# choutilin/makani

Hardware: AMD Instinct MI355X
Metric: SFNO fwd+bwd samples/sec, 73ch 721x1440 (higher is better)
Workload: dtype bf16; 1 GPU; sfno_linear_73chq_sc3_layers8_edim384 fwd+bwd+Adam, 73ch 721x1440, per-GPU batch 1; global_batch=1, parallelism=h1, spectral_dtype=f32 (GEMMs as 6 bf16 MFMA products of exact 3-way operand splits), step_launch=eager, micro_batches=1, python_gc=disabled in the timed region, adam=after backward

## Files before the change

### include/makani_amd.h

```cpp
#ifndef MAKANI_AMD_H
#define MAKANI_AMD_H

#include <stdint.h>

#ifdef __cplusplus
extern "C" {
#endif

int mk_version(void);
const char* mk_last_error(void);


int mk_quadrature(int grid, int nlat, double* theta, double* weights);

int mk_legendre_kpad(int nlat);

int mk_legendre_table(int grid, int nlat, int lmax, int mmax, int with_quad_weights, float* out);

int mk_fft_twiddle_len(int nlon);
int mk_fft_twiddles(int nlon, float* out);

int mk_rfft(const void* x, int x_dtype, float* xf, const float* twiddles,
            int bc, int nlat, int nlon, int mmax, float scale0, float scale_m, float scale_h,
            void* stream);
// ... 23 lines not shown
                          int mmax_loc, int m_off, int mmax_glob, int xf_layout, void* stream);
int mk_legendre_inv_x3_ex(const float* c, const void* tab_x3, float* xf, int bc, int nlat, int lmax,
                          int mmax_loc, int m_off, int mmax_glob, int xf_layout, void* stream);

int mk_rfft_pm(const void* x, int x_dtype, float* xf, const float* twiddles, int bc, int nlat, int nlon, int mmax,
               float scale0, float scale_m, float scale_h, int chans, int chans_per_peer, void* stream);
int mk_irfft_pm(const float* xf, void* x, int x_dtype, const float* twiddles, int bc, int nlat, int nlon, int mmax,
                float scale0, float scale_m, float scale_h, int chans, int chans_per_peer, void* stream);

int mk_irfft_sums(const float* xf, void* x, int x_dtype, const float* twiddles, int bc, int nlat, int nlon, int mmax,
                  float scale0, float scale_m, float scale_h, int xf_layout, int chans, int chans_per_peer, double* rowsums,
                  void* stream);
int mk_irfft_affine_add(const float* xf, void* x, int x_dtype, const float* twiddles, int bc, int nlat, int nlon,
                        int mmax, float scale0, float scale_m, float scale_h, int xf_layout, const void* z,
                        const float* affine, void* stream);

int mk_dhconv_fwd(const float* x, const float* w, float* y, int lloc, int mloc, int batch,
                  int cin, int cout, int l_off, int m_off, void* stream);
int mk_dhconv_dgrad(const float* gy, const float* w, float* gx, int lloc, int mloc, int batch,
                    int cin, int cout, int l_off, int m_off, void* stream);
int mk_dhconv_wgrad(const float* x, const float* gy, float* gw, int lloc, int mloc, int batch,
                    int cin, int cout, int l_off, int m_off, void* stream);

int mk_dhconv_fwd_x3(const float* x, const float* w, float* y, int lloc, int mloc, int batch,
                     int cin, int cout, int l_off, int m_off, void* stream);
int mk_dhconv_dgrad_x3(const float* gy, const float* w, float* gx, int lloc, int mloc, int batch,
                       int cin, int cout, int l_off, int m_off, void* stream);
int mk_dhconv_wgrad_x3(const float* x, const float* gy, float* gw, int lloc, int mloc, int batch,
                       int cin, int cout, int l_off, int m_off, void* stream);

// ... 117 lines not shown
```

### makani_amd/_lib.py

```python
import ctypes
import os

import torch

from . import build as _build

_LIB = None

_c_int = ctypes.c_int
_c_float = ctypes.c_float
_vp = ctypes.c_void_p

SIGNATURES = {
    "mk_version": (_c_int, []),
    "mk_last_error": (ctypes.c_char_p, []),
    "mk_quadrature": (_c_int, [_c_int, _c_int, _vp, _vp]),
    "mk_legendre_kpad": (_c_int, [_c_int]),
    "mk_legendre_table": (_c_int, [_c_int, _c_int, _c_int, _c_int, _c_int, _vp]),
    "mk_fft_twiddle_len": (_c_int, [_c_int]),
    "mk_fft_twiddles": (_c_int, [_c_int, _vp]),
    "mk_rfft": (_c_int, [_vp, _c_int, _vp, _vp, _c_int, _c_int, _c_int, _c_int, _c_float, _c_float, _c_float, _vp]),
    "mk_irfft": (_c_int, [_vp, _vp, _c_int, _vp, _c_int, _c_int, _c_int, _c_int, _c_float, _c_float, _c_float, _vp]),
    "mk_legendre_fwd": (_c_int, [_vp, _vp, _vp, _c_int, _c_int, _c_int, _c_int, _c_int, _c_int, _vp]),
    "mk_legendre_inv": (_c_int, [_vp, _vp, _vp, _c_int, _c_int, _c_int, _c_int, _c_int, _c_int, _vp]),
    "mk_legendre_x3_bytes": (ctypes.c_longlong, [_c_int, _c_int, _c_int, _c_int]),
    "mk_legendre_x3_split": (_c_int, [_vp, _vp, _c_int, _c_int, _c_int, _c_int, _vp]),
    "mk_legendre_fwd_x3": (_c_int, [_vp, _vp, _vp, _c_int, _c_int, _c_int, _c_int, _c_int, _c_int, _vp]),
    "mk_legendre_inv_x3": (_c_int, [_vp, _vp, _vp, _c_int, _c_int, _c_int, _c_int, _c_int, _c_int, _vp]),
    "mk_rfft_ex": (_c_int, [_vp, _c_int, _vp, _vp, _c_int, _c_int, _c_int, _c_int, _c_float, _c_float, _c_float, _c_int, _vp]),
    "mk_irfft_ex": (_c_int, [_vp, _vp, _c_int, _vp, _c_int, _c_int, _c_int, _c_int, _c_float, _c_float, _c_float, _c_int, _vp]),
    "mk_rfft_pm": (_c_int, [_vp, _c_int, _vp, _vp, _c_int, _c_int, _c_int, _c_int, _c_float, _c_float, _c_float, _c_int, _c_int, _vp]),
    "mk_irfft_pm": (_c_int, [_vp, _vp, _c_int, _vp, _c_int, _c_int, _c_int, _c_int, _c_float, _c_float, _c_float, _c_int, _c_int, _vp]),
    "mk_irfft_sums": (_c_int, [_vp, _vp, _c_int, _vp, _c_int, _c_int, _c_int, _c_int, _c_float, _c_float, _c_float, _c_int, _c_int,
                               _c_int, _vp, _vp]),
    "mk_irfft_affine_add": (_c_int, [_vp, _vp, _c_int, _vp, _c_int, _c_int, _c_int, _c_int, _c_float, _c_float, _c_float, _c_int,
                                     _vp, _vp, _vp]),
    "mk_legendre_fwd_x3_ex": (_c_int, [_vp, _vp, _vp, _c_int, _c_int, _c_int, _c_int, _c_int, _c_int, _c_int, _vp]),
    "mk_legendre_inv_x3_ex": (_c_int, [_vp, _vp, _vp, _c_int, _c_int, _c_int, _c_int, _c_int, _c_int, _c_int, _vp]),
    "mk_dhconv_fwd": (_c_int, [_vp, _vp, _vp] + [_c_int] * 7 + [_vp]),
    "mk_dhconv_dgrad": (_c_int, [_vp, _vp, _vp] + [_c_int] * 7 + [_vp]),
    "mk_dhconv_wgrad": (_c_int, [_vp, _vp, _vp] + [_c_int] * 7 + [_vp]),
    "mk_dhconv_fwd_x3": (_c_int, [_vp, _vp, _vp] + [_c_int] * 7 + [_vp]),
    "mk_dhconv_dgrad_x3": (_c_int, [_vp, _vp, _vp] + [_c_int] * 7 + [_vp]),
    "mk_dhconv_wgrad_x3": (_c_int, [_vp, _vp, _vp] + [_c_int] * 7 + [_vp]),
    "mk_spec_mix_fwd": (_c_int, [_vp, _vp, _vp] + [_c_int] * 7 + [_vp]),
    "mk_spec_mix_dgrad": (_c_int, [_vp, _vp, _vp] + [_c_int] * 7 + [_vp]),
    "mk_spec_mix_wgrad": (_c_int, [_vp, _vp, _vp] + [_c_int] * 7 + [_vp]),
    "mk_affine_add": (_c_int, [_vp, _vp, _vp, _vp, _c_int, _c_int, ctypes.c_longlong, _vp]),
    "mk_diag_fwd": (_c_int, [_vp, _vp, _vp, _c_int, _c_int, _c_int, ctypes.c_longlong, _vp]),
    "mk_diag_dgrad": (_c_int, [_vp, _vp, _vp, _c_int, _c_int, _c_int, ctypes.c_longlong, _vp]),
    "mk_diag_wgrad": (_c_int, [_vp, _vp, _vp, _c_int, _c_int, _c_int, ctypes.c_longlong, _vp]),
# ... 92 lines not shown
```

### makani_amd/build.py

```python
import os
import shutil
import subprocess
import sys

HERE = os.path.dirname(os.path.abspath(__file__))
CSRC = os.path.join(HERE, "csrc")
LIB = os.path.join(HERE, "libmakani_amd.so")
STAMP = LIB + ".stamp"
SOURCES = ["host.cpp", "fft.hip", "gemm.hip", "gemm_x3.hip", "layout.hip", "diag.hip", "pointwise.hip", "conv_gemm.hip", "pce.hip", "pce_mlp.hip", "adam.hip", "optim.hip", "metrics.hip", "lploss.hip", "preproc.hip", "zenith.hip"]
HEADERS = ["common.h", "fft_split.h", "lds_dma.h", "pce_common.h", os.path.join("..", "..", "include", "makani_amd.h")]


def _hipcc():
    for cand in (shutil.which("hipcc"), "/opt/rocm/bin/hipcc"):
        if cand and os.path.exists(cand):
            return cand
    raise RuntimeError("hipcc not found; libmakani_amd.so cannot be built")


def have_hipcc():
    return any(c and os.path.exists(c) for c in (shutil.which("hipcc"), "/opt/rocm/bin/hipcc"))


def _source_digest():
    import hashlib
# ... 54 lines not shown
```

### makani_amd/csrc/fft.hip

```cpp
#include "common.h"
#include "../../include/makani_amd.h"

#include <hip/hip_bf16.h>
#include <cstdint>
#include <cstdlib>
#include <type_traits>
#include <utility>

namespace {

struct XfLayout {
    int sm, sk;
    int C, Cp, Bn;
    long long pstride;
};
static thread_local XfLayout g_xl = {0, 0, 0, 0, 0, 0};
static thread_local const void* g_addz = nullptr;
static thread_local const float* g_affine = nullptr;
static thread_local double* g_rowsums = nullptr;

struct XfChan {
    size_t pbase;
    int bcx0, BCx;
};
__device__ __forceinline__ XfChan xf_chan(const XfLayout& xl, int bc0, int BC) {
    XfChan c{0, bc0, BC};
    if (xl.Cp) {
        const int b = bc0 / xl.C, ch = bc0 - b * xl.C, pp = ch / xl.Cp;
        c.pbase = (size_t)pp * (size_t)xl.pstride;
        c.bcx0 = b * xl.Cp + (ch - pp * xl.Cp);
        c.BCx = xl.Bn * xl.Cp;
    }
    return c;
}


template <int I>
using IC = std::integral_constant<int, I>;

template <class F, int... Is>
__device__ __forceinline__ void static_for_impl(F&& f, std::integer_sequence<int, Is...>) {
    (f(IC<Is>{}), ...);
}
template <int N, class F>
__device__ __forceinline__ void static_for(F&& f) {
    static_for_impl(static_cast<F&&>(f), std::make_integer_sequence<int, N>{});
}

constexpr double kPi = 3.14159265358979323846264338327950288;

constexpr double cx_reduce(double x) {
    while (x > kPi) x -= 2.0 * kPi;
    while (x < -kPi) x += 2.0 * kPi;
    return x;
}
constexpr double cx_sin(double x) {
    x = cx_reduce(x);
    double term = x, sum = x;
    for (int n = 1; n < 20; ++n) {
        term *= -x * x / ((2.0 * n) * (2.0 * n + 1.0));
        sum += term;
    }
// ... 526 lines not shown
extern "C" int mk_irfft_affine_add(const float* xf, void* x, int x_dtype, const float* twiddles, int bc, int nlat, int nlon,
                                   int mmax, float scale0, float scale_m, float scale_h, int xf_layout, const void* z,
                                   const float* affine, void* stream) {
    MK_REQUIRE(z != nullptr && affine != nullptr, "null pointer");
    MK_REQUIRE(!fft_legacy() && mmax <= 241 && (nlon == 480 || nlon == 1440), "the affine-add epilogue exists in the split kernels only");
    MK_REQUIRE((((uintptr_t)z | (uintptr_t)x) & 15) == 0, "fields must be 16-byte aligned");
    MK_REQUIRE(xf_layout == 0 || xf_layout == 1, "xf_layout must be 0 ([M][K][BC]) or 1 ([K][M][BC])");
    MK_REQUIRE((240LL * (xf_layout ? 1 : nlat) + 1) * bc * 8 < (1LL << 31), "Fourier rows too large for the 32-bit gather offsets");
    g_addz = z;
    g_affine = affine;
    const int rc = mk_irfft_ex(xf, x, x_dtype, twiddles, bc, nlat, nlon, mmax, scale0, scale_m, scale_h, xf_layout, stream);
    g_addz = nullptr;
    g_affine = nullptr;
    return rc;
}
```

### makani_amd/csrc/fft_split.h

```cpp

constexpr int SH = 240;
constexpr int SP = 272;
constexpr int SNSUB = 24;
constexpr int STHREADS = 384;
constexpr int SLDS_F2 = SNSUB * SP + 96;

__device__ __forceinline__ int pair_tile(int i) {
    const int xcd = i & 7, seq = i >> 3;
    return ((((seq >> 1) << 3) + xcd) << 1) + (seq & 1);
}

__device__ __forceinline__ int sub_base(int sr, int S) { return sr * SP + 4 * (sr / S); }
__device__ __forceinline__ int phi(int i) { return i + (i >> 4); }
__device__ __forceinline__ int opaque(int v) {
    asm volatile("" : "+v"(v));
    return v;
}

template <typename T> __device__ __forceinline__ float as_stored(float v);
template <> __device__ __forceinline__ float as_stored<float>(float v) { return v; }
template <> __device__ __forceinline__ float as_stored<__hip_bfloat16>(float v) { return __bfloat162float(__float2bfloat16(v)); }

template <bool SUMS = false, typename TOut = float>
__device__ __forceinline__ void split_passes(float2* lds, int tid, int S, const float2 (&tw15)[15], float* red = nullptr) {
// ... 206 lines not shown
        const unsigned int w[4] = {u.x, u.y, u.z, u.w};
#pragma unroll
        for (int i = 0; i < 4; ++i) {
            o[2 * i] = __uint_as_float(w[i] << 16);
            o[2 * i + 1] = __uint_as_float(w[i] & 0xffff0000u);
        }
    }
    static __device__ __forceinline__ void store(__hip_bfloat16* p, const float (&o)[8]) {
        __hip_bfloat16 h[8];
#pragma unroll
        for (int i = 0; i < 8; ++i) h[i] = __float2bfloat16(o[i]);
        *reinterpret_cast<uint4*>(p) = *reinterpret_cast<const uint4*>(h);
    }
};

template <int S, typename TOut, bool WIDE, int PERSIST, bool SUMS = false, bool ADD = false>
__global__ __launch_bounds__(STHREADS, PERSIST ? 3 : 5) void irfft_split_kernel(const float2* __restrict__ xf, TOut* __restrict__ x,
                                                               const float2* __restrict__ tw, int BC, int K, int M,
                                                               float scale0, float scale_m, float scale_h, XfLayout xl,
                                                               double* __restrict__ rowsums, const TOut* __restrict__ addz,
                                                               const float* __restrict__ affine) {
    constexpr int N = 480 * S, G = SNSUB / S, HH = N / 2;
    extern __shared__ __attribute__((aligned(16))) float2 lds[];
    float* red = reinterpret_cast<float*>(lds + SLDS_F2);
    const int tid = threadIdx.x;
    const int ntile = (BC + G - 1) / G;
    const int total = ntile * K;
    const float2* tw2 = tw + HH;
    const int total16 = (total + 15) & ~15;
    auto next_valid = [&](int i) {
        while (i < total16 && pair_tile(i) >= total) i += (int)gridDim.x;
        return i;
    };
    int sched = PERSIST ? next_valid(blockIdx.x) : (int)blockIdx.x;
    if (sched >= total16) return;
    int tile = pair_tile(sched);
    if (!PERSIST && tile >= total) return;
// ... 42 lines not shown
#pragma unroll
            for (int it = 0; it < PIT; ++it) {
                const int jp = jp0 + STEP * it, j1 = SH - jp;
                const bool oa = chan_ok && jp < NPAIR && jp < M, ob = chan_ok && jp < NPAIR && j1 < M;
                xa[it] = *(oa ? base + (size_t)jp * xl.sm * xc.BCx : xf);
                xb[it] = *(ob ? base + (size_t)j1 * xl.sm * xc.BCx : xf);
            }
        }
    };
    gather(tile, tid);
  for (;;) {
    const int tl = opaque(tid);
    const int k = tile / ntile, bc0 = (tile - k * ntile) * G;
    const int jp0 = tl / G, g = tl - jp0 * G;
    const bool chan_ok = bc0 + g < BC;
#pragma unroll
    for (int it = 0; it < PIT; ++it) {
        const int jp = jp0 + STEP * it;
        if (jp >= NPAIR) continue;
        const int j1 = SH - jp;
        const float sa = (chan_ok && jp < M) ? ((jp == 0) ? scale0 : scale_m) : 0.f;
        const float sb = (chan_ok && j1 < M) ? ((j1 == HH) ? scale_h : scale_m) : 0.f;
        const float2 a0 = make_float2(sa * xa[it].x, sa * xa[it].y);
        const float2 b0 = make_float2(sb * xb[it].x, sb * xb[it].y);
        float2 wsub = it ? cmul(wfirst[0], tw2[S * STEP * it]) : wfirst[0];
        wsub.y = -wsub.y;
#pragma unroll
        for (int s = 0; s < S; ++s) {
            float2 ya = a0, yb = b0;
            if (s > 0) {
// ... 45 lines not shown
                const float2* zs = lds + sub_base(g * S + sq, S) + phi((EO / 2) * p);
#pragma unroll
                for (int h = 0; h < EO / 2; ++h) {
                    const float2 z = zs[h];
                    r[sq][2 * h] = z.x;
                    r[sq][2 * h + 1] = -z.y;
                }
            }
            const size_t doff = ((size_t)(bc0 + g) * K + k) * N + (size_t)p * EO * S;
            TOut* dst = x + doff;
            float za[S][EO];
            float ca = 0.f, cb = 0.f;
            if constexpr (ADD) {
                ca = affine[2 * (bc0 + g)];
                cb = affine[2 * (bc0 + g) + 1];
#pragma unroll
                for (int c = 0; c < S; ++c) OutVec<TOut>::load(addz + doff + c * EO, za[c]);
            }
#pragma unroll
            for (int c = 0; c < S; ++c) {
                float o[EO];
#pragma unroll
                for (int e = 0; e < EO; ++e) {
                    const int f = c * EO + e;
                    o[e] = r[f % S][f / S];
                    if constexpr (ADD) o[e] += fmaf(za[c][e], ca, cb);
                }
                OutVec<TOut>::store(dst + c * EO, o);
            }
        }
    }
    if (next >= total16) break;
    sched = next;
    tile = pair_tile(next);
    __syncthreads();
  }
}

static inline unsigned split_grid(long long tiles) { return (unsigned)((tiles + 15) / 16 * 16); }

static inline int fft_exp() {
    static const int v = [] { const char* e = getenv("MK_FFT_EXP"); return e ? atoi(e) : 0; }();
    return v;
}

// ... 12 lines not shown
    return 0;
}

template <int S>
int launch_irfft_split(const float* xf, void* x, int x_dtype, const float* tw, int bc, int nlat, int mmax, float s0,
                       float sm, float sh, hipStream_t st) {
    constexpr int G = SNSUB / S;
    const dim3 grid(split_grid(mk::ceil_div(bc, G) * (long long)nlat));
    const size_t lds = sizeof(float2) * SLDS_F2 + 2 * SNSUB * sizeof(float);
    const long long bcx = g_xl.Cp ? (long long)g_xl.Bn * g_xl.Cp : (long long)bc;
    const bool wide = ((long long)SH * g_xl.sm + 1) * bcx * 8 >= (1LL << 31);
#define MK_IRFFT_LAUNCH(T, W, PS, SM)                                                                                  \
    hipLaunchKernelGGL((irfft_split_kernel<S, T, W, PS, SM>), grid, dim3(STHREADS), lds, st, (const float2*)xf, (T*)x,    \
                       (const float2*)tw, bc, nlat, mmax, s0, sm, sh, g_xl, g_rowsums, (const T*)nullptr, (const float*)nullptr)
#define MK_IRFFT_PICK(T)                                                                                               \
    if (g_addz) {                                                                                                      \
        if (wide) return -1;                                                                                           \
        hipLaunchKernelGGL((irfft_split_kernel<S, T, false, 0, false, true>), grid, dim3(STHREADS), lds, st,           \
                           (const float2*)xf, (T*)x, (const float2*)tw, bc, nlat, mmax, s0, sm, sh, g_xl, nullptr,     \
                           (const T*)g_addz, g_affine);                                                                \
    } else if (g_rowsums) {                                                                                                   \
        if (wide) MK_IRFFT_LAUNCH(T, true, 1, true); else MK_IRFFT_LAUNCH(T, false, 0, true);                          \
    } else {                                                                                                           \
        if (wide) MK_IRFFT_LAUNCH(T, true, 1, false); else MK_IRFFT_LAUNCH(T, false, 0, false);                        \
    }
    if (x_dtype == 0) {
        MK_IRFFT_PICK(float)
    } else {
        MK_IRFFT_PICK(__hip_bfloat16)
    }
#undef MK_IRFFT_PICK
// ... 12 lines not shown
```

### makani_amd/csrc/pointwise.hip

```cpp
#include "common.h"
#include "../../include/makani_amd.h"

#include <hip/hip_bf16.h>

namespace {

constexpr int kT = 256;
constexpr int kE = 8;
constexpr int kSteps = 4;
constexpr int kChunk = kT * kE * kSteps;

template <typename T> struct IO;
template <> struct IO<float> {
    static __device__ __forceinline__ void load(const float* p, float (&v)[kE]) {
        const float4 a = reinterpret_cast<const float4*>(p)[0], b = reinterpret_cast<const float4*>(p)[1];
        v[0] = a.x; v[1] = a.y; v[2] = a.z; v[3] = a.w; v[4] = b.x; v[5] = b.y; v[6] = b.z; v[7] = b.w;
    }
    static __device__ __forceinline__ void store(float* p, const float (&v)[kE]) {
        reinterpret_cast<float4*>(p)[0] = make_float4(v[0], v[1], v[2], v[3]);
        reinterpret_cast<float4*>(p)[1] = make_float4(v[4], v[5], v[6], v[7]);
    }
    static __device__ __forceinline__ float ld1(const float* p) { return *p; }
    static __device__ __forceinline__ void st1(float* p, float v) { *p = v; }
};
// ... 5 lines not shown
        for (int i = 0; i < 4; ++i) {
            v[2 * i] = __uint_as_float(w[i] << 16);
            v[2 * i + 1] = __uint_as_float(w[i] & 0xffff0000u);
        }
    }
    static __device__ __forceinline__ void store(__hip_bfloat16* p, const float (&v)[kE]) {
        __hip_bfloat16 h[kE];
#pragma unroll
        for (int i = 0; i < kE; ++i) h[i] = __float2bfloat16(v[i]);
        *reinterpret_cast<uint4*>(p) = *reinterpret_cast<const uint4*>(h);
    }
    static __device__ __forceinline__ float ld1(const __hip_bfloat16* p) { return __bfloat162float(*p); }
    static __device__ __forceinline__ void st1(__hip_bfloat16* p, float v) { *p = __float2bfloat16(v); }
};

struct PhiPair {
    float Phi, phi;
};
__device__ __forceinline__ PhiPair normal_cdf_pdf_fast(float x) {
    const float z = fabsf(x) * 0.70710678118654752f;
    const float t = __builtin_amdgcn_rcpf(fmaf(0.3275911f, z, 1.0f));
    float q = fmaf(1.061405429f, t, -1.453152027f);
    q = fmaf(q, t, 1.421413741f);
    q = fmaf(q, t, -0.284496736f);
    q = fmaf(q, t, 0.254829592f);
    const float e = __builtin_amdgcn_exp2f(-1.4426950408889634f * z * z);
    const float half_erfc = 0.5f * q * t * e;
    PhiPair r;
    r.Phi = x < 0.f ? half_erfc : 1.0f - half_erfc;
    r.phi = 0.3989422804014327f * e;
    return r;
}
template <typename T> struct Act;
template <> struct Act<float> {
    static __device__ __forceinline__ float gelu(float z) { return 0.5f * z * (1.f + erff(z * 0.70710678118654752440f)); }
    static __device__ __forceinline__ float gelu_grad(float z) {
        return 0.5f * (1.f + erff(z * 0.70710678118654752440f)) + z * 0.39894228040143267794f * __expf(-0.5f * z * z);
    }
};
template <> struct Act<__hip_bfloat16> {
    static __device__ __forceinline__ float gelu(float z) { return z * normal_cdf_pdf_fast(z).Phi; }
    static __device__ __forceinline__ float gelu_grad(float z) {
        const PhiPair c = normal_cdf_pdf_fast(z);
        return fmaf(z, c.phi, c.Phi);
    }
};

template <typename T, class F>
__device__ __forceinline__ void for_chunk(long long P, F&& f) {
    const long long c0 = (long long)blockIdx.x * kChunk;
#pragma unroll
    for (int s = 0; s < kSteps; ++s) {
        const long long off = c0 + ((long long)s * kT + threadIdx.x) * kE;
        if (off + kE <= P)
            f(off, kE);
        else if (off < P)
            f(off, (int)(P - off));
    }
}

__device__ __forceinline__ float block_sum(float v, float* red) {
// ... 481 lines not shown
```

### makani_amd/layers.py

```python
import math
import os

import torch
import torch.nn as nn
import torch.nn.functional as F
from torch.utils.checkpoint import checkpoint


class _X3Conv(torch.autograd.Function):

    @staticmethod
    def forward(ctx, x3, w, addend):
        from . import ops
        wf = w.detach().float()
        ctx.save_for_backward(x3, wf)
        ctx.cfg = (w.dtype, addend is not None)
        return ops.conv1x1_x3(wf, x3, out=None if addend is None else addend.detach())

    @staticmethod
    def backward(ctx, gy):
        from . import ops
        x3, wf = ctx.saved_tensors
        wdt, has_addend = ctx.cfg
        gy = gy.contiguous()
# ... 287 lines not shown
        from . import ops
        x3, w, pre = ctx.saved_tensors
        (wimg_t, gbuf), ctx.step = (ctx.step or (None, None)), None
        need_gb = ctx.bias_dtype is not None and ctx.needs_input_grad[2]
        gpre, gsum = ops.gelu_backward(pre, gh.contiguous(), need_gb)
        gx = gw = gb = None
        if ctx.needs_input_grad[0]:
            gx = ops.pce_gemm(gpre, wimg_t if wimg_t is not None else ops.pce_pack(w, transpose=True), w.shape[1])
        if ctx.needs_input_grad[1]:
            gw = ops.conv1x1_wgrad_raw(gpre, x3, out=gbuf).to(w.dtype)
        if need_gb:
            gb = gsum.to(ctx.bias_dtype)
        return gx, gw, gb, None


def encoder_head(encoder, x):
    from . import ops
    mods = list(encoder.fwd)
    pat = _mlp_pattern(mods)
    if pat is None or x.dim() != 4:
        return None
    fc1, fc2 = pat
    if fc2.bias is not None or not ops.spec_mix_supported(fc2.in_channels, fc2.out_channels):
        return None
    x3 = _engine_field(x)
    if x3 is None or not ops.pce_supported_train(fc1.out_channels, fc1.in_channels):
        return None
    with torch.autocast("cuda", enabled=False):
        h = _PceConvGelu.apply(x3, fc1.weight2d(), fc1.bias, torch.is_grad_enabled())
    return h.view(x.shape[0], fc1.out_channels, x.shape[2], x.shape[3]), fc2


class _PceMLP(torch.autograd.Function):

    @staticmethod
    def forward(ctx, x3, w1, b1, w2, b2, apply_b2, want_row_sums, keep_pre=True):
        from . import ops
        if keep_pre:
            h, pre = ops.pce_gemm(x3, ops.pce_pack(w1), w1.shape[0], bias=b1, want_pre=True, gelu=True)
        else:
            h, pre = ops.pce_gemm(x3, ops.pce_pack(w1), w1.shape[0], bias=b1, gelu=True), x3.new_empty(0)
        want_row_sums = bool(want_row_sums) and w2.shape[0] <= 768
# ... 385 lines not shown
```

### makani_amd/ops.py

```python
import ctypes
import math
import os

import numpy as np
import torch

from . import _lib

GRIDS = {"equiangular": 0, "legendre-gauss": 1}


def _stream():
    return torch.cuda.current_stream().cuda_stream


def _need_cuda(*tensors):
    for t in tensors:
        if not t.is_cuda:
            raise RuntimeError("makani_amd: the spectral ops run only on a HIP device (got a CPU tensor); "
                               "there is no CPU fallback")


def quadrature(grid, nlat):
    if grid not in GRIDS:
# ... 63 lines not shown
    else:
        m, k, bc = xf.shape
    x = torch.empty(bc, k, nlon, dtype=out_dtype, device=xf.device)
    sums = torch.zeros(bc, 2, dtype=torch.float64, device=xf.device)
    _lib.check(_lib.load().mk_irfft_sums(xf.data_ptr(), x.data_ptr(), 1 if out_dtype == torch.bfloat16 else 0, twiddles.data_ptr(),
                                         bc, k, nlon, m, 1.0, 1.0, 1.0, int(bool(kmajor)), int(chans), int(cpp), sums.data_ptr(),
                                         _stream()), "mk_irfft_sums")
    return x, sums


def irfft_affine_add_supported(nlon, mmax):
    return nlon in (480, 1440) and mmax <= 241 and os.environ.get("MK_FFT_LEGACY", "0") != "1" \
        and os.environ.get("MK_IRFFT_AFFINE_ADD", "1") != "0"


def irfft_affine_add_raw(xf, twiddles, nlon, z, affine, kmajor=False):
    _need_cuda(xf, twiddles, z, affine)
    assert xf.dim() == 3 and xf.is_contiguous() and xf.dtype == torch.complex64
    if kmajor:
        k, m, bc = xf.shape
    else:
        m, k, bc = xf.shape
    assert z.is_contiguous() and z.numel() == bc * k * nlon and z.dtype in (torch.float32, torch.bfloat16)
    assert affine.dtype == torch.float32 and affine.is_contiguous() and affine.numel() == 2 * bc
    x = torch.empty_like(z)
    _lib.check(_lib.load().mk_irfft_affine_add(xf.data_ptr(), x.data_ptr(), _pw_dtype(z), twiddles.data_ptr(), bc, k, nlon, m,
                                               1.0, 1.0, 1.0, int(bool(kmajor)), z.data_ptr(), affine.data_ptr(), _stream()),
               "mk_irfft_affine_add")
    return x


def irfft_raw(xf, twiddles, nlon, s0, sm, sh, out_dtype=torch.float32, kmajor=False):
    _need_cuda(xf, twiddles)
    assert xf.dim() == 3 and xf.is_contiguous() and xf.dtype == torch.complex64
    if kmajor:
        k, m, bc = xf.shape
    else:
        m, k, bc = xf.shape
    fused = out_dtype == torch.bfloat16 and irfft_bf16_rows(nlon, m)
    x = torch.empty(bc, k, nlon, dtype=torch.bfloat16 if fused else torch.float32, device=xf.device)
    _lib.check(_lib.load().mk_irfft_ex(xf.data_ptr(), x.data_ptr(), 1 if fused else 0, twiddles.data_ptr(), bc, k, nlon, m,
                                       s0, sm, sh, int(bool(kmajor)), _stream()), "mk_irfft")
    return x if x.dtype == out_dtype else x.to(out_dtype)

# ... 472 lines not shown
        ctx.save_for_backward(twiddles)
        ctx.nlon = x.shape[-1]
        ctx.in_dtype = x.dtype
        ctx.kmajor = kmajor
        s = 2.0 * math.pi / ctx.nlon
        return rfft_raw(x, twiddles, mmax, s, s, s, kmajor)

    @staticmethod
    def backward(ctx, gxf):
        (tw,) = ctx.saved_tensors
        n = ctx.nlon
        gx = irfft_raw(gxf.contiguous(), tw, n, 2.0 * math.pi / n, math.pi / n, 2.0 * math.pi / n, ctx.in_dtype, ctx.kmajor)
        return gx, None, None, None


class _IRFFT(torch.autograd.Function):

    @staticmethod
    def forward(ctx, xf, twiddles, nlon, out_dtype, kmajor=False, want_sums=False):
        ctx.save_for_backward(twiddles)
        ctx.mmax = xf.shape[1] if kmajor else xf.shape[0]
        ctx.kmajor = kmajor
        if want_sums:
            x, sums = irfft_sums_raw(xf, twiddles, nlon, out_dtype, kmajor)
            ctx.mark_non_differentiable(sums)
            return x, sums
        return irfft_raw(xf, twiddles, nlon, 1.0, 1.0, 1.0, out_dtype, kmajor)

    @staticmethod
    def backward(ctx, gx, *_):
# ... 165 lines not shown
        gy = gy.contiguous()
        gx = gw = None
        if ctx.needs_input_grad[0]:
            gx = spec_mix_dgrad_raw(gy, wf.view(wf.shape[0], -1), batch, l_off, m_off)
        if ctx.needs_input_grad[1]:
            gw = spec_mix_wgrad_raw(x, gy, batch, l_off, m_off).view(wshape).to(wdt)
        return gx, gw, None, None, None


def spec_mix(x, w, batch, l_off=0, m_off=0):
    return _SpecMix.apply(x, w, batch, l_off, m_off)


def rfft(x, twiddles, mmax, kmajor=False):
    return _RFFT.apply(x, twiddles, mmax, kmajor)


def irfft(xf, twiddles, nlon, out_dtype=torch.float32, kmajor=False, want_sums=False):
    return _IRFFT.apply(xf, twiddles, nlon, out_dtype, kmajor, want_sums)


def rfft_pm(x, twiddles, mmax, chans, cpp):
    return _RFFTpm.apply(x, twiddles, mmax, chans, cpp)


def irfft_pm(xf, twiddles, nlon, out_dtype, chans, cpp, want_sums=False):
    return _IRFFTpm.apply(xf, twiddles, nlon, out_dtype, chans, cpp, want_sums)


def legendre_fwd(xf, table, lmax, m_off=0, kmajor=False):
# ... 426 lines not shown
```

### makani_amd/sfnonet.py

```python
import math
import os
from functools import partial

import torch
import torch.nn as nn
import torch.nn.functional as F
from torch.utils.checkpoint import checkpoint

from . import comm
from .distributed import DistributedInverseRealFFT2, DistributedInverseRealSHT, DistributedRealFFT2, DistributedRealSHT
from .layer_norm import DistributedInstanceNorm2d, DistributedLayerNorm
from .layers import (Conv1x1, DropPath, EncoderDecoder, InstanceNorm2d, InverseRealFFT2, MLP, RealFFT2, _engine_field,
                     _is_exact_gelu, _is_noop, conv_plus_instance_norm, encoder_head, spectral_skip_plus_instance_norm,
                     spectral_skip_supported)
from .sht import InverseRealSHT, RealSHT
from .spectral_convolution import FactorizedSpectralConv, SpectralAttention, SpectralConv

_ACTIVATIONS = {"relu": nn.ReLU, "gelu": nn.GELU, "silu": nn.SiLU}


def _local_shape(transform):
    if comm.get_size("spatial") > 1:
        return transform.lat_shapes[comm.get_rank("h")], transform.lon_shapes[comm.get_rank("w")]
    return transform.nlat, transform.nlon
# ... 274 lines not shown
    def _forward_features(self, x, premix=None):
        for _ in range(self.repeat_layers):
            for i, blk in enumerate(self.blocks):
                if i == 0 and premix is not None:
                    x = blk(x, premix=premix)
                else:
                    x = checkpoint(blk, x, use_reentrant=False) if self.checkpointing >= 3 else blk(x)
        return x

    def _spectral_encoder(self, x):
        blk = self.blocks[0] if len(self.blocks) else None
        if (blk is None or hasattr(self, "pos_embed") or not _is_noop(self.pos_drop) or self.checkpointing != 0
                or self.repeat_layers != 1 or not blk.filter.takes_spectral_mix() or not blk.filter.filter.scale_residual
                or hasattr(blk, "inner_skip")):
            return None
        return encoder_head(self.encoder, x)

    def _engine_arena(self, x):
        from . import ops
        from .layers import Conv1x1
        if not (x.is_cuda and x.dim() == 4 and os.environ.get("MK_ENGINE_ARENA", "1") != "0"):
            return None
        if not (x.dtype == torch.bfloat16 or (torch.is_autocast_enabled() and torch.get_autocast_dtype("cuda") == torch.bfloat16)):
            return None
        cached = self.__dict__.get("_arena")
        if cached is None:
            convs = [m for m in self.modules() if isinstance(m, Conv1x1)]
        else:
            convs = cached[0]
        ptrs = [m.weight.data_ptr() for m in convs]
        if cached is None or cached[1] != ptrs:
# ... 35 lines not shown
```

### makani_amd/sht.py

```python
import torch
import torch.nn as nn

from . import ops


class _SHTBase(nn.Module):
    def __init__(self, nlat, nlon, lmax=None, mmax=None, grid="legendre-gauss", norm="ortho", csphase=True):
        super().__init__()
        if norm != "ortho" or not csphase:
            raise NotImplementedError("only norm='ortho', csphase=True (what Makani uses) are built")
        if grid not in ops.GRIDS:
            raise ValueError(f"Unknown quadrature mode {grid}")
        if nlon % 2:
            raise ValueError("nlon must be even")
        self.nlat, self.nlon, self.grid = nlat, nlon, grid
        self.norm, self.csphase = norm, csphase
        self.lmax = lmax or nlat
        self.mmax = mmax or nlon // 2 + 1
        if self.mmax > nlon // 2 + 1:
            raise ValueError("mmax exceeds nlon // 2 + 1")
        self.register_buffer("twiddles", ops.fft_twiddles(nlon), persistent=False)

    def _flatten(self, x, inner):
        lead = x.shape[:-2]
        bc = 1
        for s in lead:
            bc *= s
        return lead, x.reshape(bc, *inner)

    def extra_repr(self):
        return f"nlat={self.nlat}, nlon={self.nlon}, lmax={self.lmax}, mmax={self.mmax}, grid={self.grid}"


class RealSHT(_SHTBase):

    def __init__(self, nlat, nlon, lmax=None, mmax=None, grid="legendre-gauss", norm="ortho", csphase=True):
        super().__init__(nlat, nlon, lmax, mmax, grid, norm, csphase)
        self.register_buffer("weights", ops.legendre_table(grid, nlat, self.lmax, self.mmax, True), persistent=False)

    def forward_packed(self, x3):
        km = ops.SPECTRAL_GEMM == "bf16x3"
        xf = ops.rfft(x3, self.twiddles, self.mmax, km)
        return ops.legendre_fwd(xf, self.weights, self.lmax, 0, km)

    def forward(self, x):
        if x.shape[-2] != self.nlat or x.shape[-1] != self.nlon:
            raise ValueError(f"expected [..., {self.nlat}, {self.nlon}], got {tuple(x.shape)}")
        if x.dtype not in (torch.float32, torch.bfloat16):
            x = x.float()
        lead, x3 = self._flatten(x.contiguous(), (self.nlat, self.nlon))
        c = ops.spec_unpack(self.forward_packed(x3), 0, 0)
        return c.reshape(*lead, self.lmax, self.mmax)


class InverseRealSHT(_SHTBase):

    def __init__(self, nlat, nlon, lmax=None, mmax=None, grid="legendre-gauss", norm="ortho", csphase=True):
# ... 21 lines not shown
```

### makani_amd/spectral_convolution.py

```python
import math

import torch
import torch.nn as nn

from . import comm, ops
from .contractions import get_contract_fun
from .distributed import DistributedInverseRealFFT2, DistributedInverseRealSHT, DistributedRealSHT
from .sht import InverseRealSHT, RealSHT


def _is_hip_pair(fwd, inv):
    return isinstance(fwd, (RealSHT, DistributedRealSHT)) and isinstance(inv, (InverseRealSHT, DistributedInverseRealSHT))


class SpectralConv(nn.Module):
    def __init__(self, forward_transform, inverse_transform, in_channels, out_channels, operator_type="diagonal",
                 separable=False, bias=False, gain=1.0):
        super().__init__()
        self.forward_transform = forward_transform
        self.inverse_transform = inverse_transform
        self.in_channels = in_channels
        self.out_channels = out_channels
        self.modes_lat = self.inverse_transform.lmax
        self.modes_lon = self.inverse_transform.mmax
# ... 69 lines not shown
    def synthesise(self, c, B, odt):
        it = self.inverse_transform
        return it.inverse_packed(c, B, odt) if self._distributed else it.inverse_packed(c, odt)

    def residual_from_spectrum(self, c, B, dtype):
        with torch.autocast(device_type="cuda", enabled=False):
            r = self.synthesise(c, B, dtype if dtype in (torch.float32, torch.bfloat16) else torch.float32)
        return r.view(B, -1, r.shape[-2], r.shape[-1]).to(dtype)

    def takes_spectral_mix(self):
        return type(self) is SpectralConv and self._fused

    def _forward_fused(self, x, dtype, want_row_sums=False, premix=None, spectrum_residual=False):
        B, C = x.shape[0], x.shape[1]
        ft, it = self.forward_transform, self.inverse_transform
        xin = x if x.dtype in (torch.float32, torch.bfloat16) else x.float()
        xin = xin.contiguous()
        if isinstance(ft, DistributedRealSHT):
            c = ft.forward_packed(xin)
        else:
            c = ft.forward_packed(xin.view(B * C, xin.shape[2], xin.shape[3]))
        if premix is not None:
            c = ops.spec_mix(c, premix.weight, B, self.l_off, self.m_off)
            C = premix.out_channels
        odt = dtype if dtype in (torch.float32, torch.bfloat16) else torch.float32
        residual = x
        if self.scale_residual and spectrum_residual:
            residual = c
        elif self.scale_residual:
            r = self.synthesise(c, B, odt)
            residual = r.view(B, C, r.shape[-2], r.shape[-1]).to(dtype)
        y = ops.dhconv(c, self._weight_tensor(), B, self.l_off, self.m_off)
        sums = None
        if want_row_sums:
            out, sums = it.inverse_packed(y, B, odt, True) if self._distributed else it.inverse_packed(y, odt, True)
        else:
# ... 188 lines not shown
```

Measured before the change: 24.18 samples/s.

## Fuse encoder GELU gradient into iRFFT epilogue and fork RFFT skip-gradient add

Adds an iRFFT split-kernel epilogue that multiplies the synthesized gradient by the GELU derivative of the saved pre-activation and reduces per-channel bias-gradient sums. The encoder head's first conv+GELU output then feeds the first block's RFFT directly, and the backward produces gpre in one pass instead of a separate iRFFT, GELU-backward and bias reduction. A second path, rfft_fork, folds the residual skip gradient into the iRFFT via the existing affine-add epilogue for non-rescaling blocks. This saves full-resolution field reads and writes and some launches, at the cost of more template instantiations and extra per-workgroup atomics.

```diff
diff --git a/include/makani_amd.h b/include/makani_amd.h
--- a/include/makani_amd.h
+++ b/include/makani_amd.h
@@ -61,6 +61,8 @@
 int mk_irfft_affine_add(const float* xf, void* x, int x_dtype, const float* twiddles, int bc, int nlat, int nlon,
                         int mmax, float scale0, float scale_m, float scale_h, int xf_layout, const void* z,
                         const float* affine, void* stream);
+int mk_irfft_gelu_mul(const float* xf, const void* pre, void* gpre, double* rowsums, int x_dtype, const float* twiddles, int bc,
+                      int nlat, int nlon, int mmax, float scale0, float scale_m, float scale_h, int xf_layout, void* stream);
 
 int mk_dhconv_fwd(const float* x, const float* w, float* y, int lloc, int mloc, int batch,
                   int cin, int cout, int l_off, int m_off, void* stream);
diff --git a/makani_amd/_lib.py b/makani_amd/_lib.py
--- a/makani_amd/_lib.py
+++ b/makani_amd/_lib.py
@@ -35,6 +35,8 @@
                                _c_int, _vp, _vp]),
     "mk_irfft_affine_add": (_c_int, [_vp, _vp, _c_int, _vp, _c_int, _c_int, _c_int, _c_int, _c_float, _c_float, _c_float, _c_int,
                                      _vp, _vp, _vp]),
+    "mk_irfft_gelu_mul": (_c_int, [_vp, _vp, _vp, _vp, _c_int, _vp, _c_int, _c_int, _c_int, _c_int, _c_float, _c_float, _c_float,
+                                   _c_int, _vp]),
     "mk_legendre_fwd_x3_ex": (_c_int, [_vp, _vp, _vp, _c_int, _c_int, _c_int, _c_int, _c_int, _c_int, _c_int, _vp]),
     "mk_legendre_inv_x3_ex": (_c_int, [_vp, _vp, _vp, _c_int, _c_int, _c_int, _c_int, _c_int, _c_int, _c_int, _vp]),
     "mk_dhconv_fwd": (_c_int, [_vp, _vp, _vp] + [_c_int] * 7 + [_vp]),
diff --git a/makani_amd/build.py b/makani_amd/build.py
--- a/makani_amd/build.py
+++ b/makani_amd/build.py
@@ -8,7 +8,7 @@
 LIB = os.path.join(HERE, "libmakani_amd.so")
 STAMP = LIB + ".stamp"
 SOURCES = ["host.cpp", "fft.hip", "gemm.hip", "gemm_x3.hip", "layout.hip", "diag.hip", "pointwise.hip", "conv_gemm.hip", "pce.hip", "pce_mlp.hip", "adam.hip", "optim.hip", "metrics.hip", "lploss.hip", "preproc.hip", "zenith.hip"]
-HEADERS = ["common.h", "fft_split.h", "lds_dma.h", "pce_common.h", os.path.join("..", "..", "include", "makani_amd.h")]
+HEADERS = ["act.h", "common.h", "fft_split.h", "lds_dma.h", "pce_common.h", os.path.join("..", "..", "include", "makani_amd.h")]
 
 
 def _hipcc():
diff --git a/makani_amd/csrc/act.h b/makani_amd/csrc/act.h
--- /dev/null
+++ b/makani_amd/csrc/act.h
@@ -0,0 +1,33 @@
+#pragma once
+
+struct PhiPair {
+    float Phi, phi;
+};
+__device__ __forceinline__ PhiPair normal_cdf_pdf_fast(float x) {
+    const float z = fabsf(x) * 0.70710678118654752f;
+    const float t = __builtin_amdgcn_rcpf(fmaf(0.3275911f, z, 1.0f));
+    float q = fmaf(1.061405429f, t, -1.453152027f);
+    q = fmaf(q, t, 1.421413741f);
+    q = fmaf(q, t, -0.284496736f);
+    q = fmaf(q, t, 0.254829592f);
+    const float e = __builtin_amdgcn_exp2f(-1.4426950408889634f * z * z);
+    const float half_erfc = 0.5f * q * t * e;
+    PhiPair r;
+    r.Phi = x < 0.f ? half_erfc : 1.0f - half_erfc;
+    r.phi = 0.3989422804014327f * e;
+    return r;
+}
+template <typename T> struct Act;
+template <> struct Act<float> {
+    static __device__ __forceinline__ float gelu(float z) { return 0.5f * z * (1.f + erff(z * 0.70710678118654752440f)); }
+    static __device__ __forceinline__ float gelu_grad(float z) {
+        return 0.5f * (1.f + erff(z * 0.70710678118654752440f)) + z * 0.39894228040143267794f * __expf(-0.5f * z * z);
+    }
+};
+template <> struct Act<__hip_bfloat16> {
+    static __device__ __forceinline__ float gelu(float z) { return z * normal_cdf_pdf_fast(z).Phi; }
+    static __device__ __forceinline__ float gelu_grad(float z) {
+        const PhiPair c = normal_cdf_pdf_fast(z);
+        return fmaf(z, c.phi, c.Phi);
+    }
+};
diff --git a/makani_amd/csrc/fft.hip b/makani_amd/csrc/fft.hip
--- a/makani_amd/csrc/fft.hip
+++ b/makani_amd/csrc/fft.hip
@@ -17,6 +17,7 @@
 static thread_local XfLayout g_xl = {0, 0, 0, 0, 0, 0};
 static thread_local const void* g_addz = nullptr;
 static thread_local const float* g_affine = nullptr;
+static thread_local const void* g_mulz = nullptr;
 static thread_local double* g_rowsums = nullptr;
 
 struct XfChan {
@@ -46,6 +47,8 @@
 __device__ __forceinline__ void static_for(F&& f) {
     static_for_impl(static_cast<F&&>(f), std::make_integer_sequence<int, N>{});
 }
+
+#include "act.h"
 
 constexpr double kPi = 3.14159265358979323846264338327950288;
 
@@ -602,3 +605,19 @@
     g_affine = nullptr;
     return rc;
 }
+
+extern "C" int mk_irfft_gelu_mul(const float* xf, const void* pre, void* gpre, double* rowsums, int x_dtype, const float* twiddles,
+                                 int bc, int nlat, int nlon, int mmax, float scale0, float scale_m, float scale_h, int xf_layout,
+                                 void* stream) {
+    MK_REQUIRE(pre != nullptr, "null pointer");
+    MK_REQUIRE(!fft_legacy() && mmax <= 241 && (nlon == 480 || nlon == 1440), "the GELU-gradient epilogue exists in the split kernels only");
+    MK_REQUIRE((((uintptr_t)pre | (uintptr_t)gpre) & 15) == 0, "fields must be 16-byte aligned");
+    MK_REQUIRE(xf_layout == 0 || xf_layout == 1, "xf_layout must be 0 ([M][K][BC]) or 1 ([K][M][BC])");
+    MK_REQUIRE((240LL * (xf_layout ? 1 : nlat) + 1) * bc * 8 < (1LL << 31), "Fourier rows too large for the 32-bit gather offsets");
+    g_mulz = pre;
+    g_rowsums = rowsums;
+    const int rc = mk_irfft_ex(xf, gpre, x_dtype, twiddles, bc, nlat, nlon, mmax, scale0, scale_m, scale_h, xf_layout, stream);
+    g_mulz = nullptr;
+    g_rowsums = nullptr;
+    return rc;
+}
diff --git a/makani_amd/csrc/fft_split.h b/makani_amd/csrc/fft_split.h
--- a/makani_amd/csrc/fft_split.h
+++ b/makani_amd/csrc/fft_split.h
@@ -244,13 +244,14 @@
     }
 };
 
-template <int S, typename TOut, bool WIDE, int PERSIST, bool SUMS = false, bool ADD = false>
+template <int S, typename TOut, bool WIDE, int PERSIST, bool SUMS = false, bool ADD = false, bool MUL = false>
 __global__ __launch_bounds__(STHREADS, PERSIST ? 3 : 5) void irfft_split_kernel(const float2* __restrict__ xf, TOut* __restrict__ x,
                                                                const float2* __restrict__ tw, int BC, int K, int M,
                                                                float scale0, float scale_m, float scale_h, XfLayout xl,
                                                                double* __restrict__ rowsums, const TOut* __restrict__ addz,
                                                                const float* __restrict__ affine) {
     constexpr int N = 480 * S, G = SNSUB / S, HH = N / 2;
+    static_assert(!(MUL && (SUMS || ADD)), "one epilogue per instantiation");
     extern __shared__ __attribute__((aligned(16))) float2 lds[];
     float* red = reinterpret_cast<float*>(lds + SLDS_F2);
     const int tid = threadIdx.x;
@@ -323,6 +324,7 @@
     const int k = tile / ntile, bc0 = (tile - k * ntile) * G;
     const int jp0 = tl / G, g = tl - jp0 * G;
     const bool chan_ok = bc0 + g < BC;
+    if (MUL && tl < G) red[tl] = 0.f;
 #pragma unroll
     for (int it = 0; it < PIT; ++it) {
         const int jp = jp0 + STEP * it;
@@ -398,9 +400,12 @@
             if constexpr (ADD) {
                 ca = affine[2 * (bc0 + g)];
                 cb = affine[2 * (bc0 + g) + 1];
+            }
+            if constexpr (ADD || MUL) {
 #pragma unroll
                 for (int c = 0; c < S; ++c) OutVec<TOut>::load(addz + doff + c * EO, za[c]);
             }
+            float psum = 0.f;
 #pragma unroll
             for (int c = 0; c < S; ++c) {
                 float o[EO];
@@ -409,10 +414,19 @@
                     const int f = c * EO + e;
                     o[e] = r[f % S][f / S];
                     if constexpr (ADD) o[e] += fmaf(za[c][e], ca, cb);
+                    if constexpr (MUL) {
+                        o[e] *= Act<TOut>::gelu_grad(za[c][e]);
+                        psum += o[e];
+                    }
                 }
                 OutVec<TOut>::store(dst + c * EO, o);
             }
-        }
+            if constexpr (MUL) __hip_atomic_fetch_add(&red[g], psum, __ATOMIC_RELAXED, __HIP_MEMORY_SCOPE_WORKGROUP);
+        }
+    }
+    if constexpr (MUL) {
+        __syncthreads();
+        if (rowsums != nullptr && tl < G && bc0 + tl < BC) atomicAdd(&rowsums[bc0 + tl], (double)red[tl]);
     }
     if (next >= total16) break;
     sched = next;
@@ -455,7 +469,12 @@
     hipLaunchKernelGGL((irfft_split_kernel<S, T, W, PS, SM>), grid, dim3(STHREADS), lds, st, (const float2*)xf, (T*)x,    \
                        (const float2*)tw, bc, nlat, mmax, s0, sm, sh, g_xl, g_rowsums, (const T*)nullptr, (const float*)nullptr)
 #define MK_IRFFT_PICK(T)                                                                                               \
-    if (g_addz) {                                                                                                      \
+    if (g_mulz) {                                                                                                      \
+        if (wide) return -1;                                                                                           \
+        hipLaunchKernelGGL((irfft_split_kernel<S, T, false, 0, false, false, true>), grid, dim3(STHREADS), lds, st,    \
+                           (const float2*)xf, (T*)x, (const float2*)tw, bc, nlat, mmax, s0, sm, sh, g_xl, g_rowsums,   \
+                           (const T*)g_mulz, (const float*)nullptr);                                                   \
+    } else if (g_addz) {                                                                                                      \
         if (wide) return -1;                                                                                           \
         hipLaunchKernelGGL((irfft_split_kernel<S, T, false, 0, false, true>), grid, dim3(STHREADS), lds, st,           \
                            (const float2*)xf, (T*)x, (const float2*)tw, bc, nlat, mmax, s0, sm, sh, g_xl, nullptr,     \
diff --git a/makani_amd/csrc/pointwise.hip b/makani_amd/csrc/pointwise.hip
--- a/makani_amd/csrc/pointwise.hip
+++ b/makani_amd/csrc/pointwise.hip
@@ -43,37 +43,7 @@
     static __device__ __forceinline__ void st1(__hip_bfloat16* p, float v) { *p = __float2bfloat16(v); }
 };
 
-struct PhiPair {
-    float Phi, phi;
-};
-__device__ __forceinline__ PhiPair normal_cdf_pdf_fast(float x) {
-    const float z = fabsf(x) * 0.70710678118654752f;
-    const float t = __builtin_amdgcn_rcpf(fmaf(0.3275911f, z, 1.0f));
-    float q = fmaf(1.061405429f, t, -1.453152027f);
-    q = fmaf(q, t, 1.421413741f);
-    q = fmaf(q, t, -0.284496736f);
-    q = fmaf(q, t, 0.254829592f);
-    const float e = __builtin_amdgcn_exp2f(-1.4426950408889634f * z * z);
-    const float half_erfc = 0.5f * q * t * e;
-    PhiPair r;
-    r.Phi = x < 0.f ? half_erfc : 1.0f - half_erfc;
-    r.phi = 0.3989422804014327f * e;
-    return r;
-}
-template <typename T> struct Act;
-template <> struct Act<float> {
-    static __device__ __forceinline__ float gelu(float z) { return 0.5f * z * (1.f + erff(z * 0.70710678118654752440f)); }
-    static __device__ __forceinline__ float gelu_grad(float z) {
-        return 0.5f * (1.f + erff(z * 0.70710678118654752440f)) + z * 0.39894228040143267794f * __expf(-0.5f * z * z);
-    }
-};
-template <> struct Act<__hip_bfloat16> {
-    static __device__ __forceinline__ float gelu(float z) { return z * normal_cdf_pdf_fast(z).Phi; }
-    static __device__ __forceinline__ float gelu_grad(float z) {
-        const PhiPair c = normal_cdf_pdf_fast(z);
-        return fmaf(z, c.phi, c.Phi);
-    }
-};
+#include "act.h"
 
 template <typename T, class F>
 __device__ __forceinline__ void for_chunk(long long P, F&& f) {
diff --git a/makani_amd/layers.py b/makani_amd/layers.py
--- a/makani_amd/layers.py
+++ b/makani_amd/layers.py
@@ -325,7 +325,55 @@
         return gx, gw, gb, None
 
 
-def encoder_head(encoder, x):
+class _PceConvGeluRFFT(torch.autograd.Function):
+
+    @staticmethod
+    def forward(ctx, x3, w, bias, twiddles, mmax, kmajor, nlat, nlon):
+        from . import ops
+        h, pre = ops.pce_gemm(x3, ops.pce_pack(w), w.shape[0], bias=bias, want_pre=True, gelu=True)
+        ctx.save_for_backward(x3, w, pre, twiddles)
+        ctx.bias_dtype = None if bias is None else bias.dtype
+        ctx.cfg = (bool(kmajor), nlat, nlon)
+        ctx.step = _step_items(w)
+        s = 2.0 * math.pi / nlon
+        return ops.rfft_raw(h.view(h.shape[0] * h.shape[1], nlat, nlon), twiddles, mmax, s, s, s, kmajor)
+
+    @staticmethod
+    def backward(ctx, gxf):
+        from . import ops
+        x3, w, pre, tw = ctx.saved_tensors
+        kmajor, nlat, n = ctx.cfg
+        (wimg_t, gbuf), ctx.step = (ctx.step or (None, None)), None
+        need_gb = ctx.bias_dtype is not None and ctx.needs_input_grad[2]
+        gpre, gsum = ops.irfft_gelu_mul_raw(gxf.contiguous(), tw, n, pre, need_gb, kmajor,
+                                            (2.0 * math.pi / n, math.pi / n, 2.0 * math.pi / n))
+        gx = gw = gb = None
+        if ctx.needs_input_grad[0]:
+            gx = ops.pce_gemm(gpre, wimg_t if wimg_t is not None else ops.pce_pack(w, transpose=True), w.shape[1])
+        if ctx.needs_input_grad[1]:
+            gw = ops.conv1x1_wgrad_raw(gpre, x3, out=gbuf).to(w.dtype)
+        if need_gb:
+            gs = gsum.view(pre.shape[0], pre.shape[1])
+            gb = (gs[0] if gs.shape[0] == 1 else gs.sum(0)).to(ctx.bias_dtype)
+        return gx, gw, gb, None, None, None, None, None
+
+
+class EncoderHeadField:
+
+    def __init__(self, x3, fc1, shape):
+        self.x3, self.fc1, self.shape = x3, fc1, torch.Size(shape)
+        self.dtype, self.is_cuda, self.device = x3.dtype, x3.is_cuda, x3.device
+
+    def dim(self):
+        return len(self.shape)
+
+    def fourier_rows(self, twiddles, mmax, kmajor):
+        with torch.autocast("cuda", enabled=False):
+            return _PceConvGeluRFFT.apply(self.x3, self.fc1.weight2d(), self.fc1.bias, twiddles, mmax, kmajor,
+                                          self.shape[2], self.shape[3])
+
+
+def encoder_head(encoder, x, rows_for=None):
     from . import ops
     mods = list(encoder.fwd)
     pat = _mlp_pattern(mods)
@@ -337,6 +385,9 @@
     x3 = _engine_field(x)
     if x3 is None or not ops.pce_supported_train(fc1.out_channels, fc1.in_channels):
         return None
+    if (rows_for is not None and torch.is_grad_enabled() and (x.shape[2], x.shape[3]) == (rows_for.nlat, rows_for.nlon)
+            and ops.irfft_gelu_mul_supported(rows_for.nlon, rows_for.mmax)):
+        return EncoderHeadField(x3, fc1, (x.shape[0], fc1.out_channels, x.shape[2], x.shape[3])), fc2
     with torch.autocast("cuda", enabled=False):
         h = _PceConvGelu.apply(x3, fc1.weight2d(), fc1.bias, torch.is_grad_enabled())
     return h.view(x.shape[0], fc1.out_channels, x.shape[2], x.shape[3]), fc2
diff --git a/makani_amd/ops.py b/makani_amd/ops.py
--- a/makani_amd/ops.py
+++ b/makani_amd/ops.py
@@ -101,7 +101,7 @@
         and os.environ.get("MK_IRFFT_AFFINE_ADD", "1") != "0"
 
 
-def irfft_affine_add_raw(xf, twiddles, nlon, z, affine, kmajor=False):
+def irfft_affine_add_raw(xf, twiddles, nlon, z, affine, kmajor=False, scales=(1.0, 1.0, 1.0)):
     _need_cuda(xf, twiddles, z, affine)
     assert xf.dim() == 3 and xf.is_contiguous() and xf.dtype == torch.complex64
     if kmajor:
@@ -112,9 +112,30 @@
     assert affine.dtype == torch.float32 and affine.is_contiguous() and affine.numel() == 2 * bc
     x = torch.empty_like(z)
     _lib.check(_lib.load().mk_irfft_affine_add(xf.data_ptr(), x.data_ptr(), _pw_dtype(z), twiddles.data_ptr(), bc, k, nlon, m,
-                                               1.0, 1.0, 1.0, int(bool(kmajor)), z.data_ptr(), affine.data_ptr(), _stream()),
-               "mk_irfft_affine_add")
+                                               scales[0], scales[1], scales[2], int(bool(kmajor)), z.data_ptr(), affine.data_ptr(),
+                                               _stream()), "mk_irfft_affine_add")
     return x
+
+
+def irfft_gelu_mul_supported(nlon, mmax):
+    return nlon in (480, 1440) and mmax <= 241 and os.environ.get("MK_FFT_LEGACY", "0") != "1" \
+        and os.environ.get("MK_IRFFT_GELU_MUL", "1") != "0"
+
+
+def irfft_gelu_mul_raw(xf, twiddles, nlon, pre, want_row_sums=False, kmajor=False, scales=(1.0, 1.0, 1.0)):
+    _need_cuda(xf, twiddles, pre)
+    assert xf.dim() == 3 and xf.is_contiguous() and xf.dtype == torch.complex64
+    if kmajor:
+        k, m, bc = xf.shape
+    else:
+        m, k, bc = xf.shape
+    assert pre.is_contiguous() and pre.numel() == bc * k * nlon and pre.dtype in (torch.float32, torch.bfloat16)
+    gpre = torch.empty_like(pre)
+    sums = torch.zeros(bc, dtype=torch.float64, device=xf.device) if want_row_sums else None
+    _lib.check(_lib.load().mk_irfft_gelu_mul(xf.data_ptr(), pre.data_ptr(), gpre.data_ptr(), 0 if sums is None else sums.data_ptr(),
+                                             _pw_dtype(pre), twiddles.data_ptr(), bc, k, nlon, m, scales[0], scales[1], scales[2],
+                                             int(bool(kmajor)), _stream()), "mk_irfft_gelu_mul")
+    return gpre, sums
 
 
 def irfft_raw(xf, twiddles, nlon, s0, sm, sh, out_dtype=torch.float32, kmajor=False):
@@ -617,6 +638,52 @@
         return gx, None, None, None
 
 
+def rfft_fork_supported(x, nlon, mmax):
+    return x.dtype in (torch.float32, torch.bfloat16) and nlon in (480, 1440) and mmax <= 241 \
+        and os.environ.get("MK_FFT_LEGACY", "0") != "1" and os.environ.get("MK_FORK_ADD", "1") != "0"
+
+
+_UNIT_AFFINE = {}
+
+
+def _unit_affine(bc, device):
+    key = (bc, device)
+    t = _UNIT_AFFINE.get(key)
+    if t is None:
+        t = _UNIT_AFFINE[key] = torch.zeros(bc, 2, dtype=torch.float32, device=device)
+        t[:, 0].fill_(1.0)
+    return t
+
+
+class _RFFTFork(torch.autograd.Function):
+
+    @staticmethod
+    def forward(ctx, x, twiddles, mmax, kmajor=False):
+        ctx.save_for_backward(twiddles)
+        ctx.nlon = x.shape[-1]
+        ctx.in_dtype = x.dtype
+        ctx.kmajor = kmajor
+        ctx.set_materialize_grads(False)
+        s = 2.0 * math.pi / ctx.nlon
+        return rfft_raw(x, twiddles, mmax, s, s, s, kmajor), x.view_as(x)
+
+    @staticmethod
+    def backward(ctx, gxf, gskip):
+        (tw,) = ctx.saved_tensors
+        n = ctx.nlon
+        if gxf is None:
+            return gskip, None, None, None
+        scales = (2.0 * math.pi / n, math.pi / n, 2.0 * math.pi / n)
+        gxf = gxf.contiguous()
+        m = gxf.shape[1] if ctx.kmajor else gxf.shape[0]
+        if gskip is not None:
+            gskip = gskip.contiguous()
+        if gskip is not None and gskip.dtype == ctx.in_dtype and gskip.data_ptr() % 16 == 0 and rfft_fork_supported(gskip, n, m):
+            return irfft_affine_add_raw(gxf, tw, n, gskip, _unit_affine(gxf.shape[-1], gxf.device), ctx.kmajor, scales), None, None, None
+        gx = irfft_raw(gxf, tw, n, scales[0], scales[1], scales[2], ctx.in_dtype, ctx.kmajor)
+        return (gx if gskip is None else gx + gskip.reshape(gx.shape)), None, None, None
+
+
 class _IRFFT(torch.autograd.Function):
 
     @staticmethod
@@ -812,6 +879,10 @@
 
 def rfft(x, twiddles, mmax, kmajor=False):
     return _RFFT.apply(x, twiddles, mmax, kmajor)
+
+
+def rfft_fork(x, twiddles, mmax, kmajor=False):
+    return _RFFTFork.apply(x, twiddles, mmax, kmajor)
 
 
 def irfft(xf, twiddles, nlon, out_dtype=torch.float32, kmajor=False, want_sums=False):
diff --git a/makani_amd/sfnonet.py b/makani_amd/sfnonet.py
--- a/makani_amd/sfnonet.py
+++ b/makani_amd/sfnonet.py
@@ -312,7 +312,8 @@
                 or self.repeat_layers != 1 or not blk.filter.takes_spectral_mix() or not blk.filter.filter.scale_residual
                 or hasattr(blk, "inner_skip")):
             return None
-        return encoder_head(self.encoder, x)
+        ft = blk.filter.filter.forward_transform
+        return encoder_head(self.encoder, x, rows_for=ft if type(ft) is RealSHT else None)
 
     def _engine_arena(self, x):
         from . import ops
diff --git a/makani_amd/sht.py b/makani_amd/sht.py
--- a/makani_amd/sht.py
+++ b/makani_amd/sht.py
@@ -38,9 +38,12 @@
         super().__init__(nlat, nlon, lmax, mmax, grid, norm, csphase)
         self.register_buffer("weights", ops.legendre_table(grid, nlat, self.lmax, self.mmax, True), persistent=False)
 
-    def forward_packed(self, x3):
+    def forward_packed(self, x3, fork=False):
         km = ops.SPECTRAL_GEMM == "bf16x3"
-        xf = ops.rfft(x3, self.twiddles, self.mmax, km)
+        if fork:
+            xf, xr = ops.rfft_fork(x3, self.twiddles, self.mmax, km)
+            return ops.legendre_fwd(xf, self.weights, self.lmax, 0, km), xr
+        xf = x3.fourier_rows(self.twiddles, self.mmax, km) if hasattr(x3, "fourier_rows") else ops.rfft(x3, self.twiddles, self.mmax, km)
         return ops.legendre_fwd(xf, self.weights, self.lmax, 0, km)
 
     def forward(self, x):
diff --git a/makani_amd/spectral_convolution.py b/makani_amd/spectral_convolution.py
--- a/makani_amd/spectral_convolution.py
+++ b/makani_amd/spectral_convolution.py
@@ -6,6 +6,7 @@
 from . import comm, ops
 from .contractions import get_contract_fun
 from .distributed import DistributedInverseRealFFT2, DistributedInverseRealSHT, DistributedRealSHT
+from .layers import EncoderHeadField
 from .sht import InverseRealSHT, RealSHT
 
 
@@ -107,12 +108,20 @@
     def _forward_fused(self, x, dtype, want_row_sums=False, premix=None, spectrum_residual=False):
         B, C = x.shape[0], x.shape[1]
         ft, it = self.forward_transform, self.inverse_transform
-        xin = x if x.dtype in (torch.float32, torch.bfloat16) else x.float()
-        xin = xin.contiguous()
-        if isinstance(ft, DistributedRealSHT):
-            c = ft.forward_packed(xin)
-        else:
-            c = ft.forward_packed(xin.view(B * C, xin.shape[2], xin.shape[3]))
+        if isinstance(x, EncoderHeadField):
+            assert type(ft) is RealSHT and self.scale_residual
+            c = ft.forward_packed(x)
+        else:
+            xin = x if x.dtype in (torch.float32, torch.bfloat16) else x.float()
+            xin = xin.contiguous()
+            if isinstance(ft, DistributedRealSHT):
+                c = ft.forward_packed(xin)
+            elif (not self.scale_residual and xin is x and type(ft) is RealSHT
+                  and ops.rfft_fork_supported(x, ft.nlon, ft.mmax)):
+                c, xr = ft.forward_packed(xin.view(B * C, xin.shape[2], xin.shape[3]), fork=True)
+                x = xr.view(x.shape)
+            else:
+                c = ft.forward_packed(xin.view(B * C, xin.shape[2], xin.shape[3]))
         if premix is not None:
             c = ops.spec_mix(c, premix.weight, B, self.l_off, self.m_off)
             C = premix.out_channels
```

After: 24.33 samples/s, median of 6. No clear change (+0.6%).
